# terasum/mythril

Measured on AMD Instinct MI355X. Metric: constraint-evals/sec, higher is better.
Workload: dtype u32; 1 GPU; synthetic config 5: 10000 random 256-bit constraint tapes x 67108864 assignments per GPU, throughput mode; variant=plain, tapes=10000, rows_per_gpu=67108864, rows_total=67108864, vars=4, mode=count_all, engine=jit, short_circuit=True, parallelism=dp1 (row shards, all-reduce of per-tape results)

## Files before the change

mythril_amd/csrc/jit.cpp:

```cpp
#include "jit.h"

#include <stdarg.h>
#include <stdio.h>
#include <string.h>

#include <algorithm>
#include <atomic>
#include <climits>
#include <cstdlib>
#include <stdexcept>
#include <string>
#include <thread>
#include <unordered_map>
#include <vector>

namespace mh {
namespace jit {

namespace {

struct Fail {
    std::string why;
};

[[noreturn]] void fail(const std::string& w) { throw Fail{w}; }

enum LK : uint8_t { L_UNDEF, L_CONST, L_VGPR };
struct Limb {
    uint8_t k = L_UNDEF;
    uint32_t v = 0;
    static Limb C(uint32_t x) { Limb l; l.k = L_CONST; l.v = x; return l; }
    static Limb R(uint32_t r) { Limb l; l.k = L_VGPR; l.v = r; return l; }
    bool is_c() const { return k == L_CONST; }
    bool is_r() const { return k == L_VGPR; }
    bool is_c(uint32_t x) const { return k == L_CONST && v == x; }
};

struct Val {
    bool is_bool = false;
    int bconst = -1;
    int pair = -1;
    Limb l[8];
    bool defined = false;
};

enum : uint32_t { LBL_SC_SKIP = 0xFFF0, LBL_SC_END = 0xFFF1 };

constexpr uint32_t kStageMargin = 8;

int top_bit(uint32_t m) { return m ? 31 - __builtin_clz(m) : -1; }
uint32_t prefix_mask(uint32_t m) { int t = top_bit(m); return t < 0 ? 0u : ((2u << t) - 1u); }

class Emitter {
public:
    Emitter(const SsaTape& st, const std::vector<uint32_t>& pool, uint32_t n_vars,
            const Options& opt, const std::vector<uint8_t>* check = nullptr,
            std::vector<double>* insn_cost = nullptr)
        : st_(st), pool_(pool), n_vars_(n_vars), opt_(opt), check_(check),
          insn_cost_(insn_cost) {}

    TapeCode run();

private:
    SsaTape st_;
    const std::vector<uint32_t>& pool_;
    uint32_t n_vars_;
    Options opt_;
    const std::vector<uint8_t>* check_;
    std::vector<double>* insn_cost_;
    bool sc_used_ = false;
    std::vector<MI> code_;
    std::vector<Val> vals_;
    std::vector<int> last_;
    std::vector<uint8_t> dem_;
    int vref_[512] = {};
    uint32_t vbase_ = 0, vmax_ = 0, vhigh_ = 0;
    int pref_[N_BOOL_PAIRS] = {};
    uint32_t kstage_ = 0;
    uint32_t n_valu_ = 0, n_wide_ = 0, n_salu_ = 0;
    uint32_t n_valu_cold_ = 0;
    int cold_ = 0;
    bool calls_div_ = false;
    bool uses_lds_ = false;
    bool calls_kec_ = false;
    int cur_op_ = -1;
public:
    static uint64_t op_valu[256], op_wide[256], op_count[256];
private:

    void emit(uint16_t op, std::initializer_list<Opnd> ops, bool e64 = false) {
        MI m;
        m.op = op;
        m.e64 = e64 ? 1 : 0;
        m.tag = cur_op_ >= 0 ? (uint8_t)cur_op_ : 0xFF;
        int i = 0;
        for (const Opnd& o : ops) m.o[i++] = o;
        code_.push_back(m);
        if (op <= M_V_CMP_LE_F64) {
            ++n_valu_;
            if (cold_ > 0) ++n_valu_cold_;
            const bool wide = e64 || op == M_V_ADD_CO || op == M_V_ADDC_CO || op == M_V_SUB_CO ||
                              op == M_V_SUBB_CO || op == M_V_SUBREV_CO || op == M_V_SUBBREV_CO ||
                              op == M_V_OR3 || op == M_V_ALIGNBIT || op == M_V_MAD_U64_U32 ||
                              op == M_V_LSHL_ADD || op == M_V_PERM || op == M_V_BFI ||
                              op == M_V_LSHLREV || op == M_V_LSHRREV || op == M_V_ASHRREV ||
                              (op >= M_V_CMP_EQ && op <= M_V_CMP_GT_I32) || op >= M_V_CVT_F64_U32 ||
                              op == M_V_RCP_F32 || op == M_V_CMP_GT_F32 || op == M_V_CMP_LE_F32;
            if (wide) ++n_wide_;
            if (cur_op_ >= 0) { ++op_valu[cur_op_]; op_wide[cur_op_] += wide; }
        } else if (op <= M_S_CMP_LT_U32) {
            ++n_salu_;
        }
    }

    uint32_t next_lbl_ = 0x1000;

    uint32_t valloc() {
        for (uint32_t r = vbase_; r < vmax_; ++r)
            if (vref_[r] == 0) {
                vref_[r] = 1;
                vhigh_ = std::max(vhigh_, r + 1);
                return r;
            }
        fail("VGPR pressure");
    }
    uint32_t valloc_pair() {
        for (uint32_t r = (vbase_ + 1) & ~1u; r + 1 < vmax_; r += 2)
            if (vref_[r] == 0 && vref_[r + 1] == 0) {
                vref_[r] = vref_[r + 1] = 1;
                vhigh_ = std::max(vhigh_, r + 2);
                return r;
            }
        fail("VGPR pressure (pair)");
    }
    void vretain(uint32_t r) { if (r >= vbase_) ++vref_[r]; }
    void vrelease(uint32_t r) {
        if (r < vbase_) return;
        if (vref_[r] <= 0) fail("internal: VGPR refcount");
        --vref_[r];
    }

    int palloc() {
        for (int i = 0; i < (int)N_BOOL_PAIRS; ++i)
            if (pref_[i] == 0) {
                pref_[i] = 1;
                return i;
            }
        fail("SGPR pressure (Bool masks)");
    }
    static Opnd P(int i) { return S(S_BOOL0 + 2 * (uint32_t)i, 2); }

    void retain(const Val& v) {
        if (v.is_bool) {
            if (v.bconst < 0) ++pref_[v.pair];
            return;
        }
        for (const Limb& l : v.l)
            if (l.is_r()) vretain(l.v);
    }
    void release(const Val& v) {
        if (v.is_bool) {
            if (v.bconst < 0) {
                if (pref_[v.pair] <= 0) fail("internal: pair refcount");
                --pref_[v.pair];
            }
            return;
        }
        for (const Limb& l : v.l)
            if (l.is_r()) vrelease(l.v);
    }
    const Val& val(int r) const {
        if (r < 0 || r >= (int)vals_.size() || !vals_[r].defined) fail("internal: undefined vreg");
        return vals_[r];
    }
    Val const_val(int cidx) const {
        Val v;
        v.defined = true;
        for (int k = 0; k < 8; ++k) v.l[k] = Limb::C(pool_[8ull * (uint32_t)cidx + k]);
        return v;
    }
    static Val bool_const(bool b) {
        Val v;
        v.defined = true;
        v.is_bool = true;
        v.bconst = b ? 1 : 0;
        return v;
    }
    Val bool_mask(int pair) {
        Val v;
        v.defined = true;
        v.is_bool = true;
        v.pair = pair;
        return v;
    }
    int mask_of(const Val& b, std::vector<int>& tmp_pairs) {
        if (b.bconst < 0) return b.pair;
        const int p = palloc();
        tmp_pairs.push_back(p);
        emit(M_S_MOV_B64, {P(p), IMM(b.bconst ? 0xFFFFFFFFu : 0u)});
        return p;
    }

    static Opnd src(const Limb& l) {
        if (l.k == L_UNDEF) fail("internal: read of an undemanded limb");
        return l.is_c() ? IMM(l.v) : V(l.v);
    }
    uint32_t vgpr_of(const Limb& l, std::vector<uint32_t>& tmp) {
        if (l.k == L_UNDEF) fail("internal: read of an undemanded limb");
        if (l.is_r()) return l.v;
        const uint32_t t = valloc();
        tmp.push_back(t);
        emit(M_V_MOV, {V(t), IMM(l.v)});
        return t;
    }
    Opnd vi_of(const Limb& l, std::vector<uint32_t>& tmp) {
        if (l.is_c() && is_inline(l.v)) return IMM(l.v);
        return V(vgpr_of(l, tmp));
    }
    Opnd staged(uint32_t x) {
        if (is_inline(x)) return IMM(x);
        const uint32_t s = S_KSTAGE + (kstage_++ % N_KSTAGE);
        emit(M_S_MOV_B32, {S(s), IMM(x)});
        return S(s);
    }
    void free_tmp(std::vector<uint32_t>& tmp) {
        for (uint32_t r : tmp) vrelease(r);
        tmp.clear();
    }
    void free_tmp_pairs(std::vector<int>& tp) {
        for (int p : tp) --pref_[p];
        tp.clear();
    }

    int chain(bool sub, const Limb* a, const Limb* b, int top, Limb* res, uint32_t junk,
              std::vector<uint32_t>& tmp);
    void op_addsub(int d, const Val& A, const Val& B, bool sub);
    void op_logic(int d, const Val& A, const Val& B, int kind);
    Val op_eq(const Val& A, const Val& B);
    void and_all_zero(const std::vector<uint32_t>& regs, int* p, std::vector<uint32_t>& tmp);
    Val op_ult(const Val& A, const Val& B, bool signed_, bool negate);
    void op_ite(int d, const Val& C, const Val& T, const Val& E);
    Val op_bite(const Val& C, const Val& T, const Val& E);
    Val op_bool2(uint8_t op, const Val& A, const Val& B);
    void op_shr(int d, const Val& A, uint32_t s);
    void op_shl(int d, const Val& A, uint32_t s);
    void op_vshift(int d, const Val& A, const Val& B, uint8_t op);
    void op_mul(int d, const Val& A, const Val& B);
    void op_div(int d, int a, int b, int cidx, uint32_t kind, int cur);
    void rescue_div_regs(int cur, uint32_t end = R_TEMP0);
    void op_keccak(const SsaInsn& v, int cur);
    void op_exp(int d, const Val& A, const Val& E);
    void addmod_regs(const uint32_t* u, const uint32_t* v, const uint32_t* n, uint32_t* r,
                     int when = -1);
    void op_mulmod(int d, const Val& X, const Val& Y, const Val& N);
    int scratch_ = -1;
    void demand();
    template <class F> void demand_rule(const SsaInsn& v, uint32_t dd, F&& D);
    void sc_check(const Val& v);
    void emit_insn(int i, bool slice, bool no_check);
    struct Stage { int first_e, ic, acc; };
    struct Slack { uint32_t lo = 0, hi = 0; };
public:
    int stage_ = 0;
    const std::vector<uint8_t>* stage_skip_ = nullptr;
    std::vector<int> stage_rejected_;
private:
    std::vector<Stage> stages_;
    std::vector<Slack> slack_;
    std::vector<uint8_t> slack_ok_;
    bool in_slice_ = false;
    void plan_stages();
    void emit_staged(const Stage& sg);
    void cmp32(uint16_t op, Limb x, Limb y);
    bool stage_decide(const SsaInsn& c, int q, int acc);
    Val& out(int d) {
        Val& v = vals_[d];
        v = Val();
        v.defined = true;
        return v;
    }
};

int Emitter::chain(bool sub, const Limb* a, const Limb* b, int top, Limb* res, uint32_t junk,
                   std::vector<uint32_t>& tmp) {
    int cs = 0;
    uint32_t same = ~0u;
    for (int k = 0; k <= top; ++k) {
        const Limb x = a[k], y = b[k];
        if (x.k == L_UNDEF || y.k == L_UNDEF) fail("internal: chain over an undemanded limb");
        if (cs == 2 && x.is_c() && y.is_c()) {
            const bool through = sub ? x.v == y.v : (uint64_t)x.v + y.v == 0xFFFFFFFFull;
            if (through) {
                if (res) {
                    if (same == ~0u) {
                        same = valloc();
                        emit(M_V_ADDC_CO, {V(same), S(S_DIV_DUMMY, 2), IMM(sub ? 0u : ~0u),
                                           IMM(sub ? 0u : 0u), VCC()}, true);
                        if (sub) code_.back().op = M_V_SUBB_CO;
                    } else {
                        vretain(same);
                    }
                    res[k] = Limb::R(same);
                }
                continue;
            }
            same = ~0u;
            if (!res) {
                cs = sub ? (x.v < y.v ? 1 : 0) : ((uint64_t)x.v + y.v > 0xFFFFFFFFull ? 1 : 0);
                continue;
            }
            const uint32_t dst = valloc();
            if (sub) {
                if (is_inline(x.v) && is_inline(y.v))
                    emit(M_V_SUBB_CO, {V(dst), S(S_DIV_DUMMY, 2), IMM(x.v), IMM(y.v), VCC()}, true);
                else
                    emit(M_V_SUBB_CO, {V(dst), S(S_DIV_DUMMY, 2), V(vgpr_of(x, tmp)),
                                       V(vgpr_of(y, tmp)), VCC()}, true);
                cs = x.v < y.v ? 1 : 0;
            } else {
                const uint32_t sv = x.v + y.v;
                if (is_inline(sv))
                    emit(M_V_ADDC_CO, {V(dst), S(S_DIV_DUMMY, 2), IMM(sv), IMM(0), VCC()}, true);
                else
                    emit(M_V_ADDC_CO, {V(dst), S(S_DIV_DUMMY, 2), V(vgpr_of(Limb::C(sv), tmp)),
                                       IMM(0), VCC()}, true);
                cs = (uint64_t)x.v + y.v > 0xFFFFFFFFull ? 1 : 0;
            }
            res[k] = Limb::R(dst);
            continue;
        }
        same = ~0u;
// ... 798 lines not shown
    --pref_[pc];
    for (int k = 0; k < 8; ++k) {
        vrelease(sm[k]);
        vrelease(df[k]);
    }
}

void Emitter::op_mulmod(int d, const Val& X, const Val& Y, const Val& N) {
    uint32_t r[8], p[8], y[8], n[8];
    for (int k = 0; k < 8; ++k) {
        r[k] = valloc();
        emit(M_V_MOV, {V(r[k]), IMM(0)});
        p[k] = valloc();
        emit(M_V_MOV, {V(p[k]), src(X.l[k])});
        y[k] = valloc();
        emit(M_V_MOV, {V(y[k]), src(Y.l[k])});
        if (N.l[k].is_r()) {
            n[k] = N.l[k].v;
            vretain(n[k]);
        } else {
            n[k] = valloc();
            emit(M_V_MOV, {V(n[k]), src(N.l[k])});
        }
    }
    const uint32_t t = valloc();
    const int pb = palloc();
    const uint32_t top = next_lbl_++, done = next_lbl_++;
    emit(M_LABEL, {LBL(top)});
    emit(M_V_OR3, {V(t), V(y[0]), V(y[1]), V(y[2])});
    emit(M_V_OR3, {V(t), V(t), V(y[3]), V(y[4])});
    emit(M_V_OR3, {V(t), V(t), V(y[5]), V(y[6])});
    emit(M_V_OR, {V(t), V(y[7]), V(t)});
    emit(M_V_CMP_NE, {VCC(), IMM(0), V(t)});
    emit(M_S_AND_B64, {S(S_SCRATCH, 2), VCC(), S(S_VALID, 2)});
    emit(M_S_CBRANCH_SCC0, {LBL(done)});
    emit(M_V_AND, {V(t), IMM(1), V(y[0])});
    emit(M_V_CMP_NE, {P(pb), IMM(0), V(t)}, true);
    addmod_regs(r, p, n, r, pb);
    addmod_regs(p, p, n, p);
    for (int k = 0; k < 7; ++k) emit(M_V_ALIGNBIT, {V(y[k]), V(y[k + 1]), V(y[k]), IMM(1)});
    emit(M_V_LSHRREV, {V(y[7]), IMM(1), V(y[7])});
    emit(M_S_BRANCH, {LBL(top)});
    emit(M_LABEL, {LBL(done)});
    --pref_[pb];
    vrelease(t);
    for (int k = 0; k < 8; ++k) {
        vrelease(p[k]);
        vrelease(y[k]);
        vrelease(n[k]);
    }
    Val& O = out(d);
    for (int k = 0; k < 8; ++k) O.l[k] = Limb::R(r[k]);
}

void Emitter::rescue_div_regs(int cur, uint32_t end) {
    std::vector<std::pair<uint32_t, uint32_t>> moved;
    for (size_t r = 0; r < vals_.size(); ++r) {
        Val& v = vals_[r];
        if (!v.defined || v.is_bool || last_[r] <= cur) continue;
        for (Limb& l : v.l) {
            if (!l.is_r() || l.v < R_DIV0 || l.v >= end) continue;
            uint32_t nr = ~0u;
            for (auto& m : moved)
                if (m.first == l.v) nr = m.second;
            if (nr == ~0u) {
                nr = valloc();
                emit(M_V_MOV, {V(nr), V(l.v)});
                moved.push_back({l.v, nr});
            } else {
                vretain(nr);
            }
            l.v = nr;
        }
    }
}

void Emitter::op_div(int d, int a, int b, int cidx, uint32_t kind, int cur) {
    calls_div_ = true;
    rescue_div_regs(cur);
    const Val& A = val(a);
    const Val B = cidx >= 0 ? const_val(cidx) : val(b);
    if (kind >= 2 && A.l[7].is_c() && !(A.l[7].v >> 31) && B.l[7].is_c() && !(B.l[7].v >> 31))
        kind = kind == 2 ? 0u : 1u;
    if (kind < 2) {
        for (int k = 0; k < 8; ++k) emit(M_V_MOV, {V(R_DY + k), src(B.l[k])});
        for (int k = 0; k < 8; ++k) emit(M_V_MOV, {V(R_DR + k), src(A.l[k])});
    } else {
        auto sign_of = [&](const Val& X, uint32_t sreg) {
            if (X.l[7].is_c()) emit(M_V_MOV, {V(sreg), IMM((X.l[7].v >> 31) ? ~0u : 0u)});
            else emit(M_V_ASHRREV, {V(sreg), IMM(31), V(X.l[7].v)});
        };
        auto load_abs = [&](uint32_t base, uint32_t sreg, const Val& X) {
            bool allc = true;
            for (int k = 0; k < 8; ++k) allc = allc && X.l[k].is_c();
            const bool known = X.l[7].is_c(), neg = known && (X.l[7].v >> 31);
            if (allc) {
                uint32_t c[8];
                uint64_t borrow = neg ? 1 : 0;
                for (int k = 0; k < 8; ++k) {
                    const uint64_t t = (uint64_t)(neg ? ~X.l[k].v : X.l[k].v) + borrow;
                    c[k] = (uint32_t)t;
                    borrow = t >> 32;
                }
                for (int k = 0; k < 8; ++k) emit(M_V_MOV, {V(base + k), IMM(c[k])});
                return;
            }
            if (known && !neg) {
                for (int k = 0; k < 8; ++k) emit(M_V_MOV, {V(base + k), src(X.l[k])});
                return;
            }
            for (int k = 0; k < 8; ++k) {
                if (X.l[k].is_c(0)) emit(M_V_MOV, {V(base + k), V(sreg)});
                else emit(M_V_XOR, {V(base + k), src(X.l[k]), V(sreg)});
            }
            emit(M_V_SUB_CO, {V(base), VCC(), V(base), V(sreg)});
            for (int k = 1; k < 8; ++k)
                emit(M_V_SUBB_CO, {V(base + k), VCC(), V(base + k), V(sreg), VCC()});
        };
        sign_of(B, R_SY);
        sign_of(A, R_SX);
        load_abs(R_DY, R_SY, B);
        load_abs(R_DR, R_SX, A);
    }
    emit(M_S_MOV_B32, {S(S_DIV_KIND), IMM(kind)});
    emit(M_CALL_DIV, {IMM((uint32_t)code_.size())});
    Val& R = out(d);
    const uint32_t dm = dem_[d], base = kind == 1 ? R_DR : R_DQ;
    for (int k = 0; k < 8; ++k)
        if ((dm >> k) & 1) R.l[k] = Limb::R(base + k);
}

void Emitter::op_keccak(const SsaInsn& v, int cur) {
    calls_kec_ = true;
    rescue_div_regs(cur, R_TEMP_KEC);
    const uint32_t nw = (v.w1raw >> 8) & 3u, full = (v.w1raw >> 10) & 1u;
    if (nw < 1 || nw > 3) fail("keccak: bad word count");
    const int ops[3] = {v.a, v.b, v.c};
    Limb src[3][8];
    std::vector<uint32_t> tmp;
    for (uint32_t i = 0; i < nw; ++i) {
        const Val& W = val(ops[i]);
        for (int k = 0; k < 8; ++k) {
            src[i][k] = W.l[k];
            if (src[i][k].k == L_UNDEF) fail("internal: keccak over an undemanded limb");
            if (src[i][k].is_r() && src[i][k].v >= R_KEC0 && src[i][k].v < R_TEMP_KEC) {
                const uint32_t r = valloc();
                tmp.push_back(r);
                emit(M_V_MOV, {V(r), V(src[i][k].v)});
                src[i][k] = Limb::R(r);
            }
        }
    }
    emit(M_S_MOV_B32, {S(S_PERM_SEL), IMM(0x00010203u)});
    for (uint32_t i = 0; i < nw; ++i)
        for (int t = 0; t < 4; ++t)
            for (int h = 0; h < 2; ++h) {
                const uint32_t dst = R_KEC0 + 2 * (4 * i + t) + h;
                const Limb& l = src[i][h ? 6 - 2 * t : 7 - 2 * t];
                if (l.is_c()) emit(M_V_MOV, {V(dst), IMM(__builtin_bswap32(l.v))});
                else emit(M_V_PERM, {V(dst), IMM(0), V(l.v), S(S_PERM_SEL)});
            }
    free_tmp(tmp);
    for (uint32_t lane = 4 * nw; lane < 25; ++lane)
        for (uint32_t h = 0; h < 2; ++h) {
            uint32_t x = 0;
            if (full && lane == 4 * nw && h == 0) x = 1u;
            if (lane == 16 && h == 1) x = 0x80000000u;
            emit(M_V_MOV, {V(R_KEC0 + 2 * lane + h), IMM(x)});
        }
    emit(M_CALL_KEC, {IMM((uint32_t)code_.size())});
    const KecCode& kc = kec_routine();
    Val& R = out(v.d);
    const uint32_t dm = dem_[v.d];
    for (int k = 0; k < 8; ++k) {
        if (!((dm >> k) & 1)) continue;
        const uint32_t r = valloc();
        emit(M_V_PERM, {V(r), IMM(0), V(kc.out[7 - k]), S(S_PERM_SEL)});
        R.l[k] = Limb::R(r);
    }
}

template <class F>
void Emitter::demand_rule(const SsaInsn& v, uint32_t dd, F&& D) {
    const uint8_t op = v.op;
    switch (op) {
        case D_NOP: D(v.a, dd); break;
        case D_ADD_R: case D_SUB_R: case D_RSUB_R: case D_MUL_R:
            D(v.a, prefix_mask(dd));
            D(v.b, prefix_mask(dd));
            break;
        case D_AND_R: case D_OR_R: case D_XOR_R: {
            uint32_t ma = dd;
            if (v.cidx >= 0) {
                for (int k = 0; k < 8; ++k) {
                    const uint32_t c = pool_[8ull * (uint32_t)v.cidx + k];
                    if ((op == D_AND_R && c == 0) || (op == D_OR_R && c == ~0u))
                        ma &= ~(1u << k);
                }
            }
            D(v.a, ma);
            D(v.b, dd);
            break;
        }
        case D_ITE: D(v.b, dd); D(v.c, dd); break;
        case D_EXP: case D_MULMOD:
            D(v.a, 0xFF);
            D(v.b, 0xFF);
            D(v.c, 0xFF);
            break;
        case D_SHL_V: case D_LSHR_V: case D_ASHR_V:
            D(v.a, 0xFF);
            D(v.b, 0xFF);
// ... 445 lines not shown
            ask(v.a, dd, ex);
        } else if (v.op == D_ITE) {
            ask(v.b, dd, ex);
            ask(v.c, dd, ex);
        } else {
            demand_rule(v, dd, [&](int r, uint32_t m) { ask(r, m, true); });
        }
    }
    const uint32_t hot0 = n_valu_ - n_valu_cold_;
    std::vector<uint8_t> saved(sg.ic - sg.first_e);
    slack_.assign(nv, Slack());
    in_slice_ = true;
    for (int j = sg.first_e; j < sg.ic; ++j) {
        const SsaInsn& v = st_.code[j];
        saved[j - sg.first_e] = dem_[v.d];
        dem_[v.d] = sd[v.d];
        const bool is_val = !(is_compare(v.op) || (v.op >= D_BAND && v.op <= D_FALSE) ||
                              v.op == D_BITE);
        if (is_val && sd[v.d] == 0) {
            out(v.d);
            continue;
        }
        emit_insn(j, true, true);
        const Slack a = v.a >= 0 ? slack_[v.a] : Slack();
        const Slack b = v.cidx < 0 && v.b >= 0 ? slack_[v.b] : Slack();
        Slack r;
        if (slack_ok_[v.d]) {
            if (v.op == D_ADD_R) { r.lo = a.lo + b.lo; r.hi = a.hi + b.hi + 1; }
            else if (v.op == D_SUB_R) { r.lo = a.lo + b.hi + 1; r.hi = a.hi + b.lo; }
            else { r.lo = b.lo + a.hi + 1; r.hi = b.hi + a.lo; }
        } else if (v.op == D_NOP) {
            r = a;
        } else if (v.op == D_ITE) {
            const Slack t = slack_[v.b], e = slack_[v.c];
            r.lo = std::max(t.lo, e.lo);
            r.hi = std::max(t.hi, e.hi);
        }
        slack_[v.d] = r;
    }
    in_slice_ = false;
    cur_op_ = c.op;
    const bool decided = stage_decide(c, q, sg.acc);
    uint32_t l_cold = 0, l_join = 0;
    if (decided) {
        l_join = next_lbl_++;
        if (eq) {
            emit(M_S_CBRANCH_SCC0, {LBL(l_join)});
        } else {
            l_cold = next_lbl_++;
            emit(M_S_CBRANCH_SCC1, {LBL(l_cold)});
            const uint8_t k = (uint8_t)((c.op - D_ULT_R) >> 1);
            const bool swap = (k & 3) == 1 || (k & 3) == 2, negate = (k & 3) >= 2, signed_ = k >= 4;
            const Val A0 = val(c.a);
            const Val B0 = c.cidx >= 0 ? const_val(c.cidx) : val(c.b);
            const Limb x = (swap ? B0 : A0).l[7], y = (swap ? A0 : B0).l[7];
            cmp32(signed_ ? M_V_CMP_LT_I32 : M_V_CMP_LT, x, y);
            emit(negate ? M_S_NOT_B64 : M_S_MOV_B64, {P(q), VCC()});
            emit(M_S_BRANCH, {LBL(l_join)});
            emit(M_LABEL, {LBL(l_cold)});
        }
    }
    const uint32_t hot = (n_valu_ - n_valu_cold_) - hot0;
    for (int j = sg.first_e; j < sg.ic; ++j) {
        const SsaInsn& v = st_.code[j];
        if (vals_[v.d].defined) release(vals_[v.d]);
        vals_[v.d] = Val();
        dem_[v.d] = saved[j - sg.first_e];
    }
    const uint32_t full0 = n_valu_ - n_valu_cold_;
    for (int j = sg.first_e; j <= sg.ic; ++j) emit_insn(j, false, true);
    const uint32_t full = (n_valu_ - n_valu_cold_) - full0;
    n_valu_cold_ += full;
    const Val r = vals_[c.d];
    cur_op_ = c.op;
    if (r.bconst >= 0) {
        emit(M_S_MOV_B64, {P(q), IMM(r.bconst ? 0xFFFFFFFFu : 0u)});
    } else {
        emit(M_S_MOV_B64, {P(q), P(r.pair)});
        release(r);
    }
    if (decided) emit(M_LABEL, {LBL(l_join)});
    vals_[c.d] = bool_mask(q);
    if (!decided || hot + kStageMargin > full) stage_rejected_.push_back(c.d);
    if (check_ && (*check_)[c.d]) sc_check(vals_[c.d]);
}

void Emitter::emit_insn(int i, bool slice, bool no_check) {
    const SsaInsn& v = st_.code[i];
    const uint8_t op = v.op;
    cur_op_ = op;
    const uint32_t valu_before = n_valu_, cold_before = n_valu_cold_;
    ++op_count[op];
    auto Y = [&]() -> Val { return v.cidx >= 0 ? const_val(v.cidx) : val(v.b); };
    switch (op) {
        case D_NOP: {
            const Val& a = val(v.a);
            retain(a);
            vals_[v.d] = a;
            break;
        }
        case D_LOADC: vals_[v.d] = const_val(v.cidx); break;
        case D_LOADVAR: {
            const uint32_t dm = dem_[v.d];
            Val& R = out(v.d);
            for (int k = 0; k < 8; ++k)
                if ((dm >> k) & 1u) {
                    const uint32_t r = valloc();
                    emit(M_LOADCOL, {V(r), IMM(8u * v.aux + (uint32_t)k)});
                    R.l[k] = Limb::R(r);
                }
            if (dm) emit(M_S_WAITCNT_VM, {IMM(0)});
            break;
        }
        case D_TRUE: vals_[v.d] = bool_const(true); break;
        case D_FALSE: vals_[v.d] = bool_const(false); break;
        case D_ADD_R: op_addsub(v.d, val(v.a), Y(), false); break;
        case D_SUB_R: op_addsub(v.d, val(v.a), Y(), true); break;
        case D_RSUB_R: op_addsub(v.d, Y(), val(v.a), true); break;
        case D_AND_R: op_logic(v.d, val(v.a), Y(), 0); break;
        case D_OR_R: op_logic(v.d, val(v.a), Y(), 1); break;
        case D_XOR_R: op_logic(v.d, val(v.a), Y(), 2); break;
        case D_EQ_R: vals_[v.d] = op_eq(val(v.a), Y()); break;
        case D_ULT_R: vals_[v.d] = op_ult(val(v.a), Y(), false, false); break;
        case D_UGE_R: vals_[v.d] = op_ult(val(v.a), Y(), false, true); break;
        case D_UGT_R: vals_[v.d] = op_ult(Y(), val(v.a), false, false); break;
        case D_ULE_R: vals_[v.d] = op_ult(Y(), val(v.a), false, true); break;
        case D_SLT_R: vals_[v.d] = op_ult(val(v.a), Y(), true, false); break;
        case D_SGE_R: vals_[v.d] = op_ult(val(v.a), Y(), true, true); break;
        case D_SGT_R: vals_[v.d] = op_ult(Y(), val(v.a), true, false); break;
        case D_SLE_R: vals_[v.d] = op_ult(Y(), val(v.a), true, true); break;
        case D_BAND: case D_BOR: case D_BXOR: case D_BEQ:
            vals_[v.d] = op_bool2(op, val(v.a), val(v.b));
            break;
        case D_BNOT: {
            const Val& a = val(v.a);
            if (a.bconst >= 0) {
                vals_[v.d] = bool_const(!a.bconst);
            } else {
                const int p = palloc();
                emit(M_S_NOT_B64, {P(p), P(a.pair)});
                vals_[v.d] = bool_mask(p);
            }
            break;
        }
        case D_ITE: op_ite(v.d, val(v.a), val(v.b), val(v.c)); break;
        case D_BITE: vals_[v.d] = op_bite(val(v.a), val(v.b), val(v.c)); break;
        case D_MUL_R: op_mul(v.d, val(v.a), Y()); break;
        case D_SHL_V: case D_LSHR_V: case D_ASHR_V:
            op_vshift(v.d, val(v.a), val(v.b), op);
            break;
        case D_UDIV_R: case D_UREM_R: case D_SDIV_R: case D_SREM_R: case D_SMOD_R:
            op_div(v.d, v.a, v.b, v.cidx, (uint32_t)(op - D_UDIV_R) >> 1, i);
            break;
        case D_KECCAK: op_keccak(v, i); break;
        case D_EXP: op_exp(v.d, val(v.a), Y()); break;
        case D_MULMOD: op_mulmod(v.d, val(v.a), val(v.b), val(v.c)); break;
        default:
            if (op >= D_SHR0 && op <= D_SHR7) {
                const uint32_t s = 32u * (op - D_SHR0) + (v.aux & 31u);
                if (s == 0) { const Val& a = val(v.a); retain(a); vals_[v.d] = a; }
                else op_shr(v.d, val(v.a), s);
            } else if (op >= D_SHL0 && op <= D_SHL7) {
                const uint32_t p = op - D_SHL0, f = v.aux & 31u;
                const uint32_t s = f ? 32u * p + 32u - f : 32u * (p + 1u);
                if (s >= 256) {
                    Val& R = out(v.d);
                    for (int k = 0; k < 8; ++k) R.l[k] = Limb::C(0);
                } else {
                    op_shl(v.d, val(v.a), s);
                }
            } else {
                fail("op " + std::to_string(op) + " not in the JIT");
            }
            break;
    }
    vals_[v.d].defined = true;
    int seen[3] = {-1, -1, -1};
    int ns = 0;
    for (int r : {v.a, v.b, v.c}) {
        if (slice || r < 0 || last_[r] != i) continue;
        bool dup = false;
        for (int j = 0; j < ns; ++j) dup |= seen[j] == r;
        if (dup) continue;
        seen[ns++] = r;
        release(vals_[r]);
    }
    if (check_ && !slice && !no_check && (*check_)[v.d]) sc_check(vals_[v.d]);
    if (insn_cost_ && !slice) {
        const bool call = op >= D_UDIV_R && op <= D_SMOD_C;
        (*insn_cost_)[i] = (double)(n_valu_ - valu_before) -
                           (double)(n_valu_cold_ - cold_before) + (call ? 90.0 : 0.0) +
                           (op == D_KECCAK ? 7000.0 : 0.0);
    }
}

TapeCode Emitter::run() {
    TapeCode tc;
    tc.alg_ops = st_.alg_ops;
    try {
        if (check_ && stage_ > 0) plan_stages();
        const auto& code = st_.code;
        const int nv = st_.n_vregs;
        if (insn_cost_) insn_cost_->assign(code.size(), 0.0);
        const uint32_t n_pin = pinned_cols(n_vars_);
        if (st_.n_pinned != (int)n_pin) fail("assignment columns not pinned as the module pins them");
        bool has_div = false, has_kec = false;
        for (const SsaInsn& v : code) {
            if (v.op == D_KECCAK) { has_kec = true; continue; }
            if (v.op == D_LOADVAR || v.op == D_EXP) continue;
            if (v.op == D_MULMOD && (v.aux & 2u)) continue;
            if (v.op >= D_FIRST_COMPLEX) {
                fail(v.op == D_EXP ? "EXP with a symbolic exponent (interpreter only)"
                     : v.op == D_MULMOD ? "MULMOD (interpreter only)"
                                        : "complex op (interpreter only)");
            }
            if (v.op >= D_UDIV_R && v.op <= D_SMOD_C) has_div = true;
        }
        vbase_ = has_kec ? R_TEMP_KEC : has_div ? R_TEMP0 : n_pin ? R_TEMP_NODIV : R_COL0;
        vmax_ = std::min<uint32_t>(has_kec ? std::max(opt_.max_vgpr, opt_.max_vgpr_keccak)
                                           : opt_.max_vgpr, 256);
        if (vmax_ <= vbase_ + 16) fail("VGPR budget too small");
        vhigh_ = R_COL0 + 8 * n_pin;
        vals_.assign(nv, Val());
        for (int c = 0; c < st_.n_pinned; ++c) {
            Val& v = vals_[c];
            v.defined = true;
            for (int k = 0; k < 8; ++k) v.l[k] = Limb::R(R_COL0 + 8u * (uint32_t)c + k);
        }
        last_.assign(nv, -1);
        for (int i = 0; i < (int)code.size(); ++i)
            for (int r : {code[i].a, code[i].b, code[i].c})
                if (r >= 0) last_[r] = i;
        if (st_.root >= 0) last_[st_.root] = INT_MAX;
        demand();
        scratch_ = nv;
        vals_.push_back(Val());
        last_.push_back(-1);
        dem_.push_back(0xFF);
        size_t si = 0;
        for (int i = 0; i < (int)code.size(); ++i) {
            if (si < stages_.size() && stages_[si].first_e == i) {
                emit_staged(stages_[si]);
                i = stages_[si++].ic;
                continue;
            }
            emit_insn(i, false, false);
        }
        const Val& root = val(st_.root);
        tc.root_bool = root.is_bool;
        if (root.is_bool) {
            if (root.bconst >= 0) emit(M_S_MOV_B64, {S(S_RES, 2), IMM(root.bconst ? ~0u : 0u)});
            else emit(M_S_MOV_B64, {S(S_RES, 2), P(root.pair)});
            if (sc_used_) {
                emit(M_S_BRANCH, {LBL(LBL_SC_END)});
                emit(M_LABEL, {LBL(LBL_SC_SKIP)});
                emit(M_S_MOV_B64, {S(S_RES, 2), IMM(0)});
                emit(M_LABEL, {LBL(LBL_SC_END)});
            }
            for (int k = 0; k < 8; ++k) { tc.root_limbs[k] = ~0u; tc.root_const[k] = 0; }
        } else {
            uint32_t acc = ~0u, cacc = 0;
            for (int k = 0; k < 8; ++k) {
                const Limb l = root.l[k];
                if (l.is_c()) { cacc |= l.v; tc.root_limbs[k] = ~0u; tc.root_const[k] = l.v; continue; }
                tc.root_limbs[k] = l.v;
                tc.root_const[k] = 0;
                if (acc == ~0u) { acc = valloc(); emit(M_V_MOV, {V(acc), V(l.v)}); }
                else emit(M_V_OR, {V(acc), V(l.v), V(acc)});
            }
            if (cacc) emit(M_S_MOV_B64, {S(S_RES, 2), IMM(~0u)});
// ... 1277 lines not shown
    const bool valu = m.op <= M_V_CMP_LE_F64 &&
                      !(m.op >= M_V_CMP_EQ && m.op <= M_V_CMP_GT_I32) && m.op != M_V_CMP_LE_F64 &&
                      m.op != M_V_CMP_GT_F32 && m.op != M_V_CMP_LE_F32;
    const bool lds_read = m.op == M_DS_READ2ST64 || m.op == M_DS_READ_B32;
    if ((valu || lds_read) && m.o[0].k == O_V) return {m.o[0].v, m.o[0].n};
    return {0, 0};
}

bool touches(const Opnd& o, uint32_t r) { return o.k == O_V && r >= o.v && r < o.v + o.n; }

uint32_t coalesce_div_moves(std::vector<MI>& code) {
    uint32_t removed = 0;
    std::vector<char> gone(code.size(), 0);
    for (size_t p = 0; p < code.size(); ++p) {
        const MI& mv = code[p];
        if (mv.op != M_V_MOV || mv.e64 || mv.o[0].k != O_V || mv.o[0].n != 1 ||
            mv.o[1].k != O_V || mv.o[1].n != 1)
            continue;
        const uint32_t t = mv.o[0].v, x = mv.o[1].v;
        if (!((t >= R_DY && t < R_DY + 8) || (t >= R_DR && t < R_DR + 8)) || x < R_TEMP0) continue;
        size_t c = p + 1;
        while (c < code.size() && (code[c].op == M_V_MOV || code[c].op == M_S_MOV_B32)) ++c;
        if (c >= code.size() || code[c].op != M_CALL_DIV) continue;
        bool live = false;
        for (size_t f = p + 1; f < code.size() && !live; ++f) {
            if (gone[f]) continue;
            const MI& m = code[f];
            const auto w = vgpr_writes(m);
            for (int k = 0; k < 5; ++k) {
                if (w.second && k == 0) continue;
                if (touches(m.o[k], x)) live = true;
            }
            if (!live && w.second && x >= w.first && x < w.first + w.second) break;
        }
        if (live) continue;
        size_t q = p;
        bool ok = false;
        while (q-- > 0) {
            if (gone[q]) continue;
            const MI& m = code[q];
            if (m.op == M_LABEL || m.op == M_CALL_DIV || m.op == M_CALL_KEC || m.op == M_RET ||
                m.op == M_S_CBRANCH_SCC0 || m.op == M_S_CBRANCH_SCC1 || m.op == M_S_BRANCH)
                break;
            bool tt = false, pair_read = false;
            const auto w = vgpr_writes(m);
            for (int k = 0; k < 5; ++k) {
                tt |= touches(m.o[k], t);
                if (!(w.second && k == 0) && m.o[k].n > 1 && touches(m.o[k], x)) pair_read = true;
            }
            if (w.second && x >= w.first && x < w.first + w.second) {
                ok = w.second == 1 && w.first == x && !tt;
                break;
            }
            if (tt || pair_read) break;
        }
        if (!ok) continue;
        code[q].o[0].v = t;
        for (size_t i = q + 1; i < p; ++i)
            for (int k = 0; k < 5; ++k)
                if (code[i].o[k].k == O_V && code[i].o[k].n == 1 && code[i].o[k].v == x)
                    code[i].o[k].v = t;
        gone[p] = 1;
        ++removed;
    }
    if (removed) {
        std::vector<MI> out;
        out.reserve(code.size() - removed);
        for (size_t i = 0; i < code.size(); ++i)
            if (!gone[i]) out.push_back(code[i]);
        code.swap(out);
    }
    return removed;
}

}

static std::atomic<uint64_t> g_sc_fallbacks{0};

static int stage_level() {
    const char* e = std::getenv("MH_JIT_STAGE");
    return e ? std::min(3, std::max(0, atoi(e))) : 3;
}

uint64_t sc_fallbacks(bool reset) {
    return reset ? g_sc_fallbacks.exchange(0) : g_sc_fallbacks.load();
}

TapeCode emit_tape(const SsaTape& st, const std::vector<uint32_t>& pool, uint32_t n_vars,
                   const Options& opt) {
    TapeCode tc = emit_tape_body(st, pool, n_vars, opt);
    if (tc.ok && opt.coalesce) {
        const uint32_t r = coalesce_div_moves(tc.code);
        tc.n_valu -= r;
    }
    return tc;
}

TapeCode emit_tape_body(const SsaTape& st, const std::vector<uint32_t>& pool, uint32_t n_vars,
                        const Options& opt) {
    std::vector<double> cost;
    Emitter e(st, pool, n_vars, opt, nullptr, opt.short_circuit ? &cost : nullptr);
    TapeCode tc0 = e.run();
    if (opt.short_circuit) {
        SsaTape sc;
        std::vector<uint8_t> check;
        if (schedule_conjuncts(st, pool, opt.sample_rows, tc0.ok ? &cost : nullptr, sc, check)) {
            const int level = opt.stage >= 0 ? opt.stage : stage_level();
            if (level > 0) {
                Emitter e2(sc, pool, n_vars, opt, &check);
                e2.stage_ = level;
                TapeCode tc = e2.run();
                if (tc.ok && !e2.stage_rejected_.empty()) {
                    std::vector<uint8_t> skip((size_t)sc.n_vregs, 0);
                    for (int d : e2.stage_rejected_) skip[(size_t)d] = 1;
                    Emitter e3(sc, pool, n_vars, opt, &check);
                    e3.stage_ = level;
                    e3.stage_skip_ = &skip;
                    tc = e3.run();
                }
                if (tc.ok) return tc;
            }
            Emitter e2(sc, pool, n_vars, opt, &check);
            TapeCode tc = e2.run();
            if (tc.ok) return tc;
            g_sc_fallbacks.fetch_add(1, std::memory_order_relaxed);
        }
    }
    return tc0;
}

}
}
```

Before: 432.0 billion evals/s.

## Add fast paths for 256-bit division: short dividend and float small-quotient

The JIT now emits inline fast paths before the generic division call. When the dividend has fewer significant limbs than the divisor, the quotient is zero and the remainder is the dividend. For full-width unsigned or signed division, a float32 estimate of the top limbs yields the quotient when it is small and exact. The generic call runs on a cold branch only when some active lane is undecided; lanes already rejected by the short-circuit mask are excluded from that test. This adds JIT complexity and relies on the float error bounds being correct, and the new paths are controlled by the MH_JIT_DIV environment variable.

```diff
diff --git a/mythril_amd/csrc/jit.cpp b/mythril_amd/csrc/jit.cpp
--- a/mythril_amd/csrc/jit.cpp
+++ b/mythril_amd/csrc/jit.cpp
@@ -84,8 +84,10 @@
     bool uses_lds_ = false;
     bool calls_kec_ = false;
     int cur_op_ = -1;
+    int live_vreg_ = -1;
 public:
     static uint64_t op_valu[256], op_wide[256], op_count[256];
+    int div_ = 0;
 private:
 
     void emit(uint16_t op, std::initializer_list<Opnd> ops, bool e64 = false) {
@@ -247,6 +249,11 @@
     void op_vshift(int d, const Val& A, const Val& B, uint8_t op);
     void op_mul(int d, const Val& A, const Val& B);
     void op_div(int d, int a, int b, int cidx, uint32_t kind, int cur);
+    void div_undecided(Opnd decided, int cur);
+    void div_short_dividend(const Val& A, const Val& B, uint32_t kind, int nx, uint32_t dm, int cur,
+                            uint32_t l_cold);
+    void div_small_quotient(const Val& A, const Val& B, uint32_t kind, uint32_t dm, int cur,
+                            uint32_t l_cold);
     void rescue_div_regs(int cur, uint32_t end = R_TEMP0);
     void op_keccak(const SsaInsn& v, int cur);
     void op_exp(int d, const Val& A, const Val& E);
@@ -1211,6 +1218,43 @@
     const Val B = cidx >= 0 ? const_val(cidx) : val(b);
     if (kind >= 2 && A.l[7].is_c() && !(A.l[7].v >> 31) && B.l[7].is_c() && !(B.l[7].v >> 31))
         kind = kind == 2 ? 0u : 1u;
+    const uint32_t dm = dem_[d];
+    int nx = 8, ny = 8;
+    while (nx > 0 && A.l[nx - 1].is_c(0)) --nx;
+    while (ny > 0 && B.l[ny - 1].is_c(0)) --ny;
+    const uint32_t rbase = kind == 1 ? R_DR : R_DQ;
+    int path = 0;
+    if (div_ >= 1 && ny >= 1 && nx < ny && kind < 4) {
+        if (kind < 2 && B.l[ny - 1].is_c()) {
+            Val R;
+            R.defined = true;
+            for (int k = 0; k < 8; ++k) {
+                if (!((dm >> k) & 1)) continue;
+                R.l[k] = kind == 1 && k < nx ? A.l[k] : Limb::C(0);
+                if (R.l[k].is_r()) vretain(R.l[k].v);
+            }
+            vals_[d] = R;
+            return;
+        }
+        path = B.l[ny - 1].is_r() ? 1 : 0;
+        if (kind & 1)
+            for (int k = 0; k < nx; ++k)
+                if (A.l[k].is_r() && A.l[k].v >= rbase && A.l[k].v < rbase + 8 &&
+                    A.l[k].v != rbase + (uint32_t)k)
+                    path = 0;
+    } else if (div_ >= 3 && nx == 8 && ny == 8 && (kind == 0 || kind == 2)) {
+        path = 3;
+    }
+    uint32_t l_join = 0;
+    if (path) {
+        const uint32_t l_cold = next_lbl_++;
+        l_join = next_lbl_++;
+        if (path == 1) div_short_dividend(A, B, kind, nx, dm, cur, l_cold);
+        else div_small_quotient(A, B, kind, dm, cur, l_cold);
+        emit(M_S_BRANCH, {LBL(l_join)});
+        emit(M_LABEL, {LBL(l_cold)});
+        ++cold_;
+    }
     if (kind < 2) {
         for (int k = 0; k < 8; ++k) emit(M_V_MOV, {V(R_DY + k), src(B.l[k])});
         for (int k = 0; k < 8; ++k) emit(M_V_MOV, {V(R_DR + k), src(A.l[k])});
@@ -1253,10 +1297,118 @@
     }
     emit(M_S_MOV_B32, {S(S_DIV_KIND), IMM(kind)});
     emit(M_CALL_DIV, {IMM((uint32_t)code_.size())});
+    if (path) {
+        --cold_;
+        emit(M_LABEL, {LBL(l_join)});
+    }
+    const int nr = path == 1 && (kind & 1) ? nx : 8;
     Val& R = out(d);
-    const uint32_t dm = dem_[d], base = kind == 1 ? R_DR : R_DQ;
     for (int k = 0; k < 8; ++k)
-        if ((dm >> k) & 1) R.l[k] = Limb::R(base + k);
+        if ((dm >> k) & 1) R.l[k] = k < nr ? Limb::R(rbase + k) : Limb::C(0);
+}
+
+void Emitter::div_undecided(Opnd decided, int cur) {
+    const Opnd t = S(S_DIV_TM, 2);
+    emit(M_S_ANDN2_B64, {t, S(S_VALID, 2), decided});
+    const int lv = live_vreg_;
+    if (check_ && lv >= 0 && vals_[lv].defined && vals_[lv].is_bool && vals_[lv].bconst < 0 &&
+        last_[lv] > cur)
+        emit(M_S_AND_B64, {t, t, P(vals_[lv].pair)});
+}
+
+void Emitter::div_short_dividend(const Val& A, const Val& B, uint32_t kind, int nx, uint32_t dm,
+                                 int cur, uint32_t l_cold) {
+    int ny = 8;
+    while (!B.l[ny - 1].is_r()) --ny;
+    const uint32_t top = B.l[ny - 1].v;
+    if (kind < 2) {
+        emit(M_V_CMP_NE, {VCC(), IMM(0), V(top)});
+    } else {
+        emit(M_V_ASHRREV, {V(R_T1), IMM(31), V(top)});
+        emit(M_V_XOR, {V(R_T1), V(top), V(R_T1)});
+        emit(M_V_CMP_NE, {VCC(), IMM(0), V(R_T1)});
+    }
+    div_undecided(VCC(), cur);
+    emit(M_S_CBRANCH_SCC1, {LBL(l_cold)});
+    const uint32_t base = kind == 1 ? R_DR : R_DQ;
+    for (int k = 0; k < 8; ++k) {
+        if (!((dm >> k) & 1)) continue;
+        if (!(kind & 1)) {
+            emit(M_V_MOV, {V(base + k), IMM(0)});
+        } else if (k < nx && !(A.l[k].is_r() && A.l[k].v == base + (uint32_t)k)) {
+            emit(M_V_MOV, {V(base + k), src(A.l[k])});
+        }
+    }
+}
+
+void Emitter::div_small_quotient(const Val& A, const Val& B, uint32_t kind, uint32_t dm, int cur,
+                                 uint32_t l_cold) {
+    const Opnd K32 = S(S_DIV_F64K), KT = S(S_DIV_F64K + 1), ONE = S(S_DIV_YNZ);
+    const Opnd MSK = S(S_DIV_MSK, 2);
+    Opnd x7 = src(A.l[7]), x6 = src(A.l[6]), y7 = src(B.l[7]), y6 = src(B.l[6]);
+    if (kind == 2) {
+        auto tops = [&](const Val& X, uint32_t sreg, uint32_t t, Opnd& h7, Opnd& h6) {
+            if (X.l[7].is_c()) {
+                const uint32_t m = (X.l[7].v >> 31) ? ~0u : 0u;
+                emit(M_V_MOV, {V(sreg), IMM(m)});
+                if (!m) return;
+                h7 = IMM(~X.l[7].v);
+                if (X.l[6].is_c()) h6 = IMM(~X.l[6].v);
+                else { emit(M_V_NOT, {V(t + 1), V(X.l[6].v)}); h6 = V(t + 1); }
+                return;
+            }
+            emit(M_V_ASHRREV, {V(sreg), IMM(31), V(X.l[7].v)});
+            emit(M_V_XOR, {V(t), V(X.l[7].v), V(sreg)});
+            emit(M_V_XOR, {V(t + 1), src(X.l[6]), V(sreg)});
+            h7 = V(t);
+            h6 = V(t + 1);
+        };
+        tops(B, R_SY, R_MAD, y7, y6);
+        tops(A, R_SX, R_CARRY, x7, x6);
+    }
+    emit(M_S_MOV_B32, {K32, IMM(0x4f800000u)});
+    emit(M_V_CVT_F32_U32, {V(R_FT), x7});
+    emit(M_V_CVT_F32_U32, {V(R_FT + 1), x6});
+    emit(M_V_FMA_F32, {V(R_FR), V(R_FT), K32, V(R_FT + 1)});
+    emit(M_V_CVT_F32_U32, {V(R_FT), y7});
+    emit(M_V_CVT_F32_U32, {V(R_FT + 1), y6});
+    emit(M_V_FMA_F32, {V(R_FY), V(R_FT), K32, V(R_FT + 1)});
+    emit(M_V_RCP_F32, {V(R_FY), V(R_FY)});
+    emit(M_S_NOP, {IMM(1)});
+    emit(M_V_MUL_F32, {V(R_FC), V(R_FR), V(R_FY)});
+    emit(M_V_CMP_GT_F32, {VCC(), IMM(0x44800000u), V(R_FC)});
+    emit(M_S_MOV_B64, {MSK, VCC()});
+    if (y7.k == O_V) {
+        emit(M_V_CMP_NE, {VCC(), IMM(0), y7});
+        emit(M_S_AND_B64, {MSK, MSK, VCC()});
+    } else if (y7.v == 0) {
+        emit(M_S_MOV_B64, {MSK, IMM(0)});
+    }
+    emit(M_V_FRACT_F32, {V(R_FT), V(R_FC)});
+    emit(M_S_MOV_B32, {KT, IMM(0x35800000u)});
+    emit(M_V_FMA_F32, {V(R_T1), V(R_FC), KT, KT});
+    emit(M_V_CMP_GT_F32, {VCC(), V(R_T1), V(R_FT)});
+    emit(M_S_MOV_B64, {S(S_DIV_TM, 2), VCC()});
+    emit(M_V_CMP_LE_F32, {VCC(), IMM(0x3f800000u), V(R_FC)});
+    emit(M_S_AND_B64, {S(S_DIV_TM, 2), S(S_DIV_TM, 2), VCC()});
+    emit(M_S_ANDN2_B64, {MSK, MSK, S(S_DIV_TM, 2)});
+    emit(M_S_MOV_B32, {ONE, IMM(0x3f800000u)});
+    emit(M_V_FMA_F32, {V(R_T1), V(R_T1), ONE, V(R_FT)});
+    emit(M_V_CMP_LE_F32, {VCC(), IMM(0x3f800000u), V(R_T1)});
+    emit(M_S_ANDN2_B64, {MSK, MSK, VCC()});
+    div_undecided(MSK, cur);
+    emit(M_S_CBRANCH_SCC1, {LBL(l_cold)});
+    emit(M_V_CVT_U32_F32, {V(R_DQ), V(R_FC)});
+    if (kind == 2) {
+        emit(M_V_XOR, {V(R_T1), V(R_SX), V(R_SY)});
+        emit(M_V_XOR, {V(R_DQ), V(R_DQ), V(R_T1)});
+        emit(M_V_SUB_U32, {V(R_DQ), V(R_DQ), V(R_T1)});
+    }
+    for (int k = 1; k < 8; ++k) {
+        if (!((dm >> k) & 1)) continue;
+        if (kind == 2) emit(M_V_ASHRREV, {V(R_DQ + k), IMM(31), V(R_DQ)});
+        else emit(M_V_MOV, {V(R_DQ + k), IMM(0)});
+    }
 }
 
 void Emitter::op_keccak(const SsaInsn& v, int cur) {
@@ -1868,7 +2020,10 @@
     if (decided) emit(M_LABEL, {LBL(l_join)});
     vals_[c.d] = bool_mask(q);
     if (!decided || hot + kStageMargin > full) stage_rejected_.push_back(c.d);
-    if (check_ && (*check_)[c.d]) sc_check(vals_[c.d]);
+    if (check_ && (*check_)[c.d]) {
+        sc_check(vals_[c.d]);
+        live_vreg_ = c.d;
+    }
 }
 
 void Emitter::emit_insn(int i, bool slice, bool no_check) {
@@ -1971,7 +2126,10 @@
         seen[ns++] = r;
         release(vals_[r]);
     }
-    if (check_ && !slice && !no_check && (*check_)[v.d]) sc_check(vals_[v.d]);
+    if (check_ && !slice && !no_check && (*check_)[v.d]) {
+        sc_check(vals_[v.d]);
+        live_vreg_ = v.d;
+    }
     if (insn_cost_ && !slice) {
         const bool call = op >= D_UDIV_R && op <= D_SMOD_C;
         (*insn_cost_)[i] = (double)(n_valu_ - valu_before) -
@@ -3415,6 +3573,13 @@
     return e ? std::min(3, std::max(0, atoi(e))) : 3;
 }
 
+static int div_level() {
+    const char* s = std::getenv("MH_JIT_STAGE");
+    if (s && atoi(s) <= 0) return 0;
+    const char* e = std::getenv("MH_JIT_DIV");
+    return e ? std::min(3, std::max(0, atoi(e))) : 3;
+}
+
 uint64_t sc_fallbacks(bool reset) {
     return reset ? g_sc_fallbacks.exchange(0) : g_sc_fallbacks.load();
 }
@@ -3431,8 +3596,10 @@
 
 TapeCode emit_tape_body(const SsaTape& st, const std::vector<uint32_t>& pool, uint32_t n_vars,
                         const Options& opt) {
+    const int dlevel = div_level();
     std::vector<double> cost;
     Emitter e(st, pool, n_vars, opt, nullptr, opt.short_circuit ? &cost : nullptr);
+    e.div_ = opt.short_circuit ? 0 : dlevel;
     TapeCode tc0 = e.run();
     if (opt.short_circuit) {
         SsaTape sc;
@@ -3442,22 +3609,31 @@
             if (level > 0) {
                 Emitter e2(sc, pool, n_vars, opt, &check);
                 e2.stage_ = level;
+                e2.div_ = dlevel;
                 TapeCode tc = e2.run();
                 if (tc.ok && !e2.stage_rejected_.empty()) {
                     std::vector<uint8_t> skip((size_t)sc.n_vregs, 0);
                     for (int d : e2.stage_rejected_) skip[(size_t)d] = 1;
                     Emitter e3(sc, pool, n_vars, opt, &check);
                     e3.stage_ = level;
+                    e3.div_ = dlevel;
                     e3.stage_skip_ = &skip;
                     tc = e3.run();
                 }
                 if (tc.ok) return tc;
             }
             Emitter e2(sc, pool, n_vars, opt, &check);
+            e2.div_ = dlevel;
             TapeCode tc = e2.run();
             if (tc.ok) return tc;
             g_sc_fallbacks.fetch_add(1, std::memory_order_relaxed);
         }
+        if (dlevel > 0 && tc0.ok && tc0.calls_div) {
+            Emitter e4(st, pool, n_vars, opt);
+            e4.div_ = dlevel;
+            TapeCode tc = e4.run();
+            if (tc.ok) return tc;
+        }
     }
     return tc0;
 }
```

Result: faster. 457.0 billion evals/s (median of 6 runs) (+5.8%).
